# zfountas/deep-active-inference-mc

Measured on AMD Instinct MI355X. Metric: EFE rollouts/sec (64x64 dSprites, 10 MC-samples, depth 5), higher is better.
Workload: dtype f32; 1 GPU; calculate_G_repeated: 128 rows (32 roots x 4 actions) x depth 5 x 10 MC samples per GPU (BASELINE configs[1]) + action posterior; rows_per_gpu=128, samples=10, depth=5, parallelism=episodes sharded x1, weights replicated

## Files before the change

deep-active-inference-mc_amd/csrc/decoder.hip:

```cpp
#include <utility>
#include "mfma_pipe.h"

namespace efe {

template <class F, int... I> __device__ __forceinline__ void static_for_(F&& f, std::integer_sequence<int, I...>) { (f(std::integral_constant<int, I>{}), ...); }
template <int N, class F> __device__ __forceinline__ void static_for(F&& f) { static_for_(f, std::make_integer_sequence<int, N>{}); }

__host__ __device__ constexpr int w3_nch(int G) { return G == 4 ? 5 : 4; }
__host__ __device__ constexpr int w3_prod(int G, int c) {
    return G < 4 ? 5 * ((G >> 1) + 2 * (c >> 1)) + (G & 1) + 2 * (c & 1)
         : G == 4 ? (c < 2 ? 5 * (1 + 2 * c) + 4 : c < 4 ? 20 + 1 + 2 * (c - 2) : 24)
                  : (c < 2 ? 5 * (2 * c) + 4 : 20 + 2 * (c - 2));
}
__host__ __device__ constexpr bool w3_direct(int pp) { return f22_o1(pp / 5) < 0 && f22_o1(pp % 5) < 0; }
__host__ __device__ constexpr int w3_view(int pp) { return 3 * f22_view(pp / 5) + f22_view(pp % 5); }
__host__ __device__ constexpr int w3_mat(int pp) { return 4 * f22_wt(pp / 5) + f22_wt(pp % 5); }
__host__ __device__ constexpr bool w3_hits(int pp, int o) {
    const int r = o >> 2, c = o & 3, pr = pp / 5, pc = pp % 5;
    return (r == f22_o0(pr) || r == f22_o1(pr)) && (c == f22_o0(pc) || c == f22_o1(pc));
}
__host__ __device__ constexpr bool w3_seen(int G, int c, int o) {
    for (int g = 0; g < G; ++g)
        for (int k = 0; k < w3_nch(g); ++k) if (w3_hits(w3_prod(g, k), o)) return true;
    if (!w3_direct(w3_prod(G, c)))
        for (int k = 0; k < w3_nch(G); ++k)
            if ((w3_direct(w3_prod(G, k)) || k < c) && w3_hits(w3_prod(G, k), o)) return true;
    return false;
}
__host__ __device__ constexpr bool w3_uses_view(int G, int vi) {
    for (int k = 0; k < w3_nch(G); ++k) if (w3_view(w3_prod(G, k)) == vi) return true;
    return false;
}
__host__ __device__ constexpr bool f22_in(int a, int r) { return a == 0 ? r <= 1 : (a == 1 ? r == 1 : r >= 1); }
__host__ __device__ constexpr bool w3_reads(int G, int r, int c) {
    for (int vi = 0; vi < 9; ++vi) if (w3_uses_view(G, vi) && f22_in(vi / 3, r) && f22_in(vi % 3, c)) return true;
    return false;
}

constexpr int DA_PS = 17;
constexpr int DA_BIAS = 273 * DA_PS;

__host__ __device__ constexpr int wino_i0(int a) { return a == 0 ? 0 : (a == 2 ? 2 : 1); }
__host__ __device__ constexpr int wino_i1(int a) { return a == 0 ? 2 : (a == 1 ? 2 : (a == 2 ? 1 : 3)); }
__host__ __device__ constexpr float wino_s1(int a) { return a == 1 ? 1.0f : -1.0f; }
__host__ __device__ constexpr float wino_at(int r, int a) { return r == 0 ? (a < 3 ? 1.0f : 0.0f) : (a == 0 ? 0.0f : (a == 1 ? 1.0f : -1.0f)); }

template <int NR, int R0, class Pix>
__device__ __forceinline__ void wino_l1(f32x16 (&out)[NR][2], const float4* __restrict__ U, const float4* sm, const int h,
                                        const int mt_, Pix pix) {
    constexpr int PD = 4;
    const unsigned ln = (threadIdx.x & 63u) * 16u;
    const __amdgpu_buffer_rsrc_t ur = wrsrc(U);
    int mt = mt_; asm volatile("" : "+s"(mt));
    constexpr int a_lo = NR == 2 ? 0 : R0, a_hi = NR == 2 ? 4 : R0 + 3;
    auto ufrag = [&](int a, int b, int kc) { return wfrag(ur, ln, (size_t)(((4 * a + b) * 2 + mt) * 8 + kc) * 64); };
    auto bases = [&](int a, int b, int (&pb)[4]) {
        const int i0 = wino_i0(a), i1 = wino_i1(a), j0 = wino_i0(b), j1 = wino_i1(b);
        pb[0] = pix(i0, j0); pb[1] = pix(i0, j1); pb[2] = pix(i1, j0); pb[3] = pix(i1, j1);
    };
    float4 aq[PD], raw[4];
    int pb[4];
#pragma unroll
    for (int p = 0; p < PD; ++p) aq[p] = ufrag(a_lo, 0, p);
    bases(a_lo, 0, pb);
#pragma unroll
    for (int q = 0; q < 4; ++q) raw[q] = sm[pb[q] + h];
    f32x16 xacc;
    const f32x16 zero = {};
    auto otrans = [&](int a, int b, const f32x16& m, auto mask) {
        constexpr int MASK = decltype(mask)::value;
#pragma unroll
        for (int r = 0; r < NR; ++r) {
            if (!((MASK >> r) & 1)) continue;
            const float car = wino_at(R0 + r, a);
#pragma unroll
            for (int c = 0; c < 2; ++c) {
                const float cbc = wino_at(c, b);
                if (cbc == 0.0f) continue;
                const float cf = car * cbc;
#pragma unroll
                for (int e = 0; e < 16; ++e) out[r][c][e] = __builtin_fmaf(cf, m[e], out[r][c][e]);
            }
        }
    };
    auto xi_row = [&](int a, auto mask) {
        const float s1 = wino_s1(a);
        const int an = a + 1 < a_hi ? a + 1 : a;
#pragma unroll
        for (int b = 0; b < 4; ++b) {
            const float t1 = wino_s1(b);
#pragma unroll
            for (int kc = 0; kc < 8; ++kc) {
                const float4 av = aq[kc % PD];
                aq[kc % PD] = (b * 8 + kc + PD < 32) ? ufrag(a, (b * 8 + kc + PD) >> 3, (kc + PD) & 7) : ufrag(an, 0, (kc + PD) & 7);
                float4 v;
                {
                    const float4 c0 = make_float4(__builtin_fmaf(s1, raw[2].x, raw[0].x), __builtin_fmaf(s1, raw[2].y, raw[0].y),
                                                  __builtin_fmaf(s1, raw[2].z, raw[0].z), __builtin_fmaf(s1, raw[2].w, raw[0].w));
                    const float4 c1 = make_float4(__builtin_fmaf(s1, raw[3].x, raw[1].x), __builtin_fmaf(s1, raw[3].y, raw[1].y),
                                                  __builtin_fmaf(s1, raw[3].z, raw[1].z), __builtin_fmaf(s1, raw[3].w, raw[1].w));
                    v = make_float4(__builtin_fmaf(t1, c1.x, c0.x), __builtin_fmaf(t1, c1.y, c0.y), __builtin_fmaf(t1, c1.z, c0.z), __builtin_fmaf(t1, c1.w, c0.w));
                }
                if (kc < 7) {
#pragma unroll
                    for (int q = 0; q < 4; ++q) raw[q] = sm[pb[q] + 2 * (kc + 1) + h];
                } else {
                    if (b < 3) bases(a, b + 1, pb);
                    else bases(an, 0, pb);
#pragma unroll
                    for (int q = 0; q < 4; ++q) raw[q] = sm[pb[q] + h];
                }
                __builtin_amdgcn_sched_barrier(0);
                f32x16& x = xacc;
                x = __builtin_amdgcn_mfma_f32_32x32x2f32(av.x, v.x, kc == 0 ? zero : x, 0, 0, 0);
                x = __builtin_amdgcn_mfma_f32_32x32x2f32(av.y, v.y, x, 0, 0, 0);
                x = __builtin_amdgcn_mfma_f32_32x32x2f32(av.z, v.z, x, 0, 0, 0);
                x = __builtin_amdgcn_mfma_f32_32x32x2f32(av.w, v.w, x, 0, 0, 0);
            }
            otrans(a, b, xacc, mask);
        }
    };
    if constexpr (NR == 2) {
        xi_row(0, std::integral_constant<int, 1>{});
#pragma unroll 1
        for (int a = 1; a < 3; ++a) xi_row(a, std::integral_constant<int, 3>{});
        xi_row(3, std::integral_constant<int, 2>{});
    } else {
#pragma unroll 1
        for (int a = a_lo; a < a_hi; ++a) xi_row(a, std::integral_constant<int, 1>{});
    }
}
struct F22Nb { int xb, c2[3], r2; };
__device__ __forceinline__ f32x4 f22_wfrag(const __amdgpu_buffer_rsrc_t wr, const unsigned ln, int ct, int m, int kc) {
    return __builtin_bit_cast(f32x4, wfrag(wr, ln + (unsigned)kc * 1024u, (size_t)(m * 4 + ct) * 256));
}
constexpr int F22_PD = 2;
__device__ __forceinline__ void f22_l2_first(f32x4 (&aq)[F22_PD][5], const __amdgpu_buffer_rsrc_t wr, const int dn, const unsigned ln) {
    static_for<F22_PD>([&](auto p) {
        static_for<w3_nch(p >> 2)>([&](auto c) { aq[p][c] = f22_wfrag(wr, ln, dn, w3_mat(w3_prod(p >> 2, c)), p & 3); });
    });
}
__device__ __forceinline__ void f22_l2(f32x4 (&acc)[16], f32x4 (&aq)[F22_PD][5], const __amdgpu_buffer_rsrc_t wr, const int dn,
                                       const unsigned ln, const f32x4 bias4, const f32x4* smv, const F22Nb& nb) {
    constexpr int NST = 24;
    auto px = [&](int i, int jj, int kc) -> f32x4 {
        return smv[(jj == 2 ? nb.c2[i] : (i == 2 ? nb.r2 + jj * DA_PS : nb.xb + (16 * i + jj) * DA_PS)) + 4 * kc];
    };
    auto view = [&](const f32x4 (&x)[9], int vi) -> f32x4 {
        const int va = vi / 3, vb = vi % 3;
        auto cv = [&](int i) -> f32x4 { return vb == 0 ? x[3 * i] - x[3 * i + 1] : (vb == 1 ? x[3 * i + 1] : x[3 * i + 2] - x[3 * i + 1]); };
        return va == 0 ? cv(0) - cv(1) : (va == 1 ? cv(1) : cv(2) - cv(1));
    };
    const f32x4 zero4 = {};
    f32x4 tq[5], xr[9];
    static_for<9>([&](auto i) { if constexpr (w3_reads(0, i / 3, i % 3)) xr[i] = px(i / 3, i % 3, 0); });
    static_for<NST>([&](auto stc) {
        constexpr int ST = decltype(stc)::value, G = ST >> 2, KC = ST & 3, GN = (ST + 1) >> 2, KN = (ST + 1) & 3;
        constexpr int SP = (ST + F22_PD) % NST, GP = SP >> 2, KP = SP & 3;
        f32x4 vw[9], ac[5];
        static_for<9>([&](auto vi) { if constexpr (w3_uses_view(G, vi)) vw[vi] = view(xr, vi); });
#pragma unroll
        for (int c = 0; c < 5; ++c) ac[c] = aq[ST % F22_PD][c];
        static_for<w3_nch(GP)>([&](auto c) { aq[ST % F22_PD][c] = f22_wfrag(wr, ln, ST + F22_PD < NST ? 0 : dn, w3_mat(w3_prod(GP, c)), KP); });
        if constexpr (ST + 1 < NST)
            static_for<9>([&](auto i) { if constexpr (w3_reads(GN, i / 3, i % 3)) xr[i] = px(i / 3, i % 3, KN); });
        __builtin_amdgcn_sched_barrier(0);
#pragma unroll
        for (int e = 0; e < 4; ++e)
            static_for<w3_nch(G)>([&](auto c) {
                constexpr int PP = w3_prod(G, c);
                const float b = vw[w3_view(PP)][e], av = ac[c][e];
                if constexpr (w3_direct(PP)) {
                    constexpr int O = 4 * f22_o0(PP / 5) + f22_o0(PP % 5);
                    constexpr bool FIRST = KC == 0 && !w3_seen(G, c, O);
                    acc[O] = __builtin_amdgcn_mfma_f32_16x16x4f32(av, b, (FIRST && e == 0) ? bias4 : acc[O], 0, 0, 0);
                } else {
                    tq[c] = __builtin_amdgcn_mfma_f32_16x16x4f32(av, b, (KC == 0 && e == 0) ? zero4 : tq[c], 0, 0, 0);
                }
            });
        if constexpr (KC == 3)
            static_for<w3_nch(G)>([&](auto c) {
                constexpr int PP = w3_prod(G, c);
                if constexpr (!w3_direct(PP))
                    static_for<16>([&](auto o) {
                        if constexpr (w3_hits(PP, o)) {
                            if constexpr (w3_seen(G, c, o)) acc[o] = acc[o] + tq[c];
                            else acc[o] = bias4 + tq[c];
                        }
                    });
            });
    });
}
__device__ __forceinline__ void f22_l2_store(f32x4 (&acc)[16], const __amdgpu_buffer_rsrc_t yr, const unsigned yoff, const int ct, const bool on) {
#pragma unroll
    for (int orow = 0; orow < 4; ++orow)
#pragma unroll
        for (int c = 0; c < 2; ++c) {
            u32x4 lo, hi;
#pragma unroll
            for (int e = 0; e < 4; ++e) {
                const unsigned x0 = __builtin_bit_cast(unsigned, relu_nan(acc[4 * orow + c][e]));
                const unsigned x1 = __builtin_bit_cast(unsigned, relu_nan(acc[4 * orow + c + 2][e]));
                const auto sw = __builtin_amdgcn_permlane32_swap(x0, x1, false, false);
                lo[e] = sw[0]; hi[e] = sw[1];
            }
            const unsigned so = (unsigned)(((2 * (orow & 1) + c) * 4096 + 2 * ct * 512 + (orow >> 1) * 32) * 16);
            if (on) {
                __builtin_amdgcn_raw_buffer_store_b128(lo, yr, yoff, so, 0);
                __builtin_amdgcn_raw_buffer_store_b128(hi, yr, yoff, so + 512u * 16u, 0);
            }
        }
}

__global__ void __launch_bounds__(256, 2) k_dec_a(const DecAArgs a) {
    constexpr int NTHR = 256;
    constexpr int NPH = 2048 / NTHR;
    constexpr int NPE = 8;
    extern __shared__ __attribute__((aligned(16))) float4 sm[];
    const int tid = threadIdx.x;
    const int lane = tid & 63;
    const int w = __builtin_amdgcn_readfirstlane(tid >> 6);

    const float4* W1 = reinterpret_cast<const float4*>(a.w1);
    const float4* W2 = reinterpret_cast<const float4*>(a.w2);

    if ((int)blockIdx.x >= a.rows) return;
    int* const slot = reinterpret_cast<int*>(sm + DA_BIAS + 32);
    if (tid == 0) slot[0] = 2 * (int)gridDim.x + atomicAdd(a.queue, 1);
    int nimg = (int)blockIdx.x + (int)gridDim.x;
    f32x4 pf[2 * NPH];
    f32x4* smv = reinterpret_cast<f32x4*>(sm);
    {
        const f32x4* X = reinterpret_cast<const f32x4*>(a.x4) + (size_t)blockIdx.x * 4096;
#pragma unroll
        for (int it = 0; it < 2 * NPH; ++it) pf[it] = X[w * 1024 + it * 64 + lane];
    }
    for (int i = tid; i < 17 * DA_PS; i += NTHR) sm[256 * DA_PS + i] = make_float4(0.f, 0.f, 0.f, 0.f);
    if (tid < 16) sm[DA_BIAS + tid] = reinterpret_cast<const float4*>(a.b1)[tid];
    else if (tid < 32) sm[DA_BIAS + tid] = reinterpret_cast<const float4*>(a.b2)[tid - 16];

    for (int img = blockIdx.x; img < a.rows;) {
        int tl_ = tid; asm volatile("" : "+v"(tl_));
        const int j = tl_ & 31, h = (tl_ >> 5) & 1;
        const bool live = row_live(a.live, img);
        if (live) {
            const int sbase = (64 * w + ((tl_ >> 4) & 3)) * DA_PS + (tl_ & 15);
#pragma unroll
            for (int it = 0; it < 2 * NPH; ++it) smv[sbase + it * 4 * DA_PS] = pf[it];
        }
        __syncthreads();
        const int nnimg = slot[0];
        int ticket = 0;
        if (tid == 0) ticket = 2 * (int)gridDim.x + atomicAdd(a.queue, 1);
        const int l1mt = w >> 1, l1n = 32 * (w & 1) + j;
        const int l1y = 2 * (l1n >> 3) - 1, l1x = 2 * (l1n & 7) - 1;
        if (live) {
            f32x16 l1o[2][2];
#pragma unroll
            for (int g4 = 0; g4 < 4; ++g4) {
                const float4 bb = sm[DA_BIAS + l1mt * 8 + 2 * g4 + h];
#pragma unroll
                for (int rc = 0; rc < 4; ++rc) { l1o[rc >> 1][rc & 1][4 * g4] = bb.x; l1o[rc >> 1][rc & 1][4 * g4 + 1] = bb.y; l1o[rc >> 1][rc & 1][4 * g4 + 2] = bb.z; l1o[rc >> 1][rc & 1][4 * g4 + 3] = bb.w; }
            }
            wino_l1<2, 0>(l1o, W1, sm, h, l1mt, [&](int i, int jj) {
                const int y = l1y + i, x = l1x + jj;
                return ((unsigned)y < 16u && (unsigned)x < 16u ? y * 16 + x : 256) * DA_PS;
            });
            __syncthreads();
            if (tid == 0) slot[0] = ticket;
#pragma unroll
            for (int rc = 0; rc < 4; ++rc) {
                const int pix = (l1y + 1 + (rc >> 1)) * 16 + l1x + 1 + (rc & 1);
#pragma unroll
                for (int g4 = 0; g4 < 4; ++g4) {
                    const f32x16& o = l1o[rc >> 1][rc & 1];
                    float4 v;
                    v.x = relu_nan(o[4 * g4 + 0]); v.y = relu_nan(o[4 * g4 + 1]);
                    v.z = relu_nan(o[4 * g4 + 2]); v.w = relu_nan(o[4 * g4 + 3]);
                    sm[pix * DA_PS + l1mt * 8 + 2 * g4 + h] = v;
                }
            }
        } else {
            __syncthreads();
            if (tid == 0) slot[0] = ticket;
        }
        __syncthreads();
        {
            int t2_ = tid; asm volatile("" : "+v"(t2_));
            const int n = t2_ & 15, g = (t2_ >> 4) & 3;
            const int bu = 2 * w + (n >> 3), bv = n & 7;
            const int zq = 256 * DA_PS + g;
            F22Nb nb;
            nb.xb = (32 * bu + 2 * bv) * DA_PS + g;
            nb.c2[0] = bv == 7 ? zq : nb.xb + 2 * DA_PS;
            nb.c2[1] = bv == 7 ? zq : nb.xb + 18 * DA_PS;
            nb.c2[2] = bv == 7 ? zq : nb.xb + 34 * DA_PS;
            nb.r2 = nb.xb + 32 * DA_PS;
            const unsigned ln = (unsigned)(t2_ & 63) * 16u;
            const unsigned yoff = (unsigned)(((32 * bu + 2 * bv + (g >> 1)) * 2 + (g & 1)) * 16);
            const __amdgpu_buffer_rsrc_t yr = wrsrc(a.y2 + (size_t)__builtin_amdgcn_readfirstlane(img) * (32 * 32 * 64));
            auto load_next = [&](const int lo, const int hi) {
                const int pimg = __builtin_amdgcn_readfirstlane(nimg < a.rows ? nimg : img);
                const __amdgpu_buffer_rsrc_t xr = wrsrc(a.x4 + (size_t)pimg * 16384);
#pragma unroll
                for (int it = 0; it < 2 * NPH; ++it)
                    if (it >= lo && it < hi) pf[it] = __builtin_bit_cast(f32x4, wfrag(xr, (unsigned)(w * 16384 + (t2_ & 63) * 16 + (it & 3) * 1024), (size_t)(it >> 2) * 256));
            };
            if (live) {
                f32x4 aq[F22_PD][5], acc2[16];
                f22_l2_first(aq, wrsrc(W2), 0, ln);
                load_next(0, NPE);
#pragma unroll 1
                for (int ct = 0; ct < 4; ++ct) {
                    const f32x4 bias4 = smv[DA_BIAS + 16 + 4 * ct + g];
                    f22_l2(acc2, aq, wrsrc(W2 + ct * 256), ct < 3 ? 1 : 0, ln, bias4, smv, nb);
                    if (ct < 3) f22_l2_store(acc2, yr, yoff, ct, true);
                }
                load_next(NPE, 2 * NPH);
                f22_l2_store(acc2, yr, yoff, 3, true);
            } else {
                load_next(0, 2 * NPH);
            }
        }
        __syncthreads();
        img = nimg; nimg = nnimg;
    }
}

constexpr int DAS_IN = 6 * 16;
constexpr int DAS_L1 = 4 * 16;
constexpr int DAS_BIAS = (DAS_IN + 1 + DAS_L1 + 2) * DA_PS;
constexpr size_t DAS_LDS_BYTES = (DAS_BIAS + 32) * sizeof(float4);
__global__ void __launch_bounds__(256, 2) k_dec_a_s(const DecAArgs a) {
    extern __shared__ __attribute__((aligned(16))) float4 sm[];
    float4* sin = sm;
    float4* sl1 = sm + (DAS_IN + 1) * DA_PS;
    const int tid = threadIdx.x, lane = tid & 63;
    const int w = __builtin_amdgcn_readfirstlane(tid >> 6);
    const int j = lane & 31, h = lane >> 5;
    const int img = blockIdx.x >> 3, p = blockIdx.x & 7;
    if (!row_live(a.live, img)) return;
    const float4* W1 = reinterpret_cast<const float4*>(a.w1);
    const float4* W2 = reinterpret_cast<const float4*>(a.w2);
    {
        const float4* X = reinterpret_cast<const float4*>(a.x4) + (size_t)img * 4096;
        const int c4 = tid & 15, px0 = tid >> 4;
        float4 v[6];
#pragma unroll
        for (int it = 0; it < 6; ++it) {
            const int pix = px0 + 16 * it, lr = pix >> 4, y = 2 * p - 1 + lr;
            v[it] = (y >= 0 && y < 16) ? X[(y * 16 + (pix & 15)) * 16 + c4] : make_float4(0.f, 0.f, 0.f, 0.f);
        }
#pragma unroll
        for (int it = 0; it < 6; ++it) sin[(px0 + 16 * it) * DA_PS + c4] = v[it];
    }
    if (tid < 16) sin[DAS_IN * DA_PS + tid] = make_float4(0.f, 0.f, 0.f, 0.f);
    if (tid < 2 * DA_PS) sl1[DAS_L1 * DA_PS + tid] = make_float4(0.f, 0.f, 0.f, 0.f);
    if (tid < 16) sm[DAS_BIAS + tid] = reinterpret_cast<const float4*>(a.b1)[tid];
    else if (tid < 32) sm[DAS_BIAS + tid] = reinterpret_cast<const float4*>(a.b2)[tid - 16];
    __syncthreads();
    const int mt = w >> 1;
    {
        const int r = w & 1, n = j & 15;
        const int ly = 2 * (n >> 3) - 1, lx = 2 * (n & 7) - 1;
        f32x16 o[1][2];
#pragma unroll
        for (int g4 = 0; g4 < 4; ++g4) {
            const float4 bb = sm[DAS_BIAS + mt * 8 + 2 * g4 + h];
#pragma unroll
            for (int c = 0; c < 2; ++c) { o[0][c][4 * g4] = bb.x; o[0][c][4 * g4 + 1] = bb.y; o[0][c][4 * g4 + 2] = bb.z; o[0][c][4 * g4 + 3] = bb.w; }
        }
        auto pix = [&](int i, int jj) {
            const int sy = ly + 1 + i, x = lx + jj, y = 2 * p - 1 + sy;
            return ((unsigned)y < 16u && (unsigned)x < 16u ? sy * 16 + x : DAS_IN) * DA_PS;
        };
        if (r) wino_l1<1, 1>(o, W1, sin, h, mt, pix);
        else wino_l1<1, 0>(o, W1, sin, h, mt, pix);
        if (j < 16)
#pragma unroll
        for (int c = 0; c < 2; ++c)
#pragma unroll
            for (int g4 = 0; g4 < 4; ++g4) {
                float4 v;
                v.x = relu_nan(o[0][c][4 * g4 + 0]); v.y = relu_nan(o[0][c][4 * g4 + 1]);
                v.z = relu_nan(o[0][c][4 * g4 + 2]); v.w = relu_nan(o[0][c][4 * g4 + 3]);
                sl1[((ly + 1 + r) * 16 + lx + 1 + c) * DA_PS + mt * 8 + 2 * g4 + h] = v;
            }
    }
    __syncthreads();
    {
        const int n = lane & 15, g = lane >> 4, bv = n & 7;
        const int zq = DAS_L1 * DA_PS + g;
        F22Nb nb;
        nb.xb = 2 * bv * DA_PS + g;
        nb.c2[0] = bv == 7 ? zq : nb.xb + 2 * DA_PS;
        nb.c2[1] = bv == 7 ? zq : nb.xb + 18 * DA_PS;
        nb.c2[2] = (bv == 7 || p == 7) ? zq : nb.xb + 34 * DA_PS;
        nb.r2 = p == 7 ? zq : nb.xb + 32 * DA_PS;
        const unsigned ln = (unsigned)lane * 16u;
        const unsigned yoff = (unsigned)(((32 * p + 2 * bv + (g >> 1)) * 2 + (g & 1)) * 16);
        const __amdgpu_buffer_rsrc_t yr = wrsrc(a.y2 + (size_t)img * (32 * 32 * 64));
        const __amdgpu_buffer_rsrc_t wr = wrsrc(W2 + w * 256);
        f32x4 aq[F22_PD][5], acc2[16];
        f22_l2_first(aq, wr, 0, ln);
        const f32x4 bias4 = reinterpret_cast<const f32x4*>(sm)[DAS_BIAS + 16 + 4 * w + g];
        f22_l2(acc2, aq, wr, 0, ln, bias4, reinterpret_cast<const f32x4*>(sl1), nb);
        f22_l2_store(acc2, yr, yoff, w, n < 8);
    }
}

constexpr size_t DA_LDS_BYTES = (DA_BIAS + 33) * sizeof(float4);
int init_dec_b_kernels();
int init_decoder_kernels() {
    if (hipFuncSetAttribute((const void*)k_dec_a, hipFuncAttributeMaxDynamicSharedMemorySize, DA_LDS_BYTES) != hipSuccess) return 1;
    if (hipFuncSetAttribute((const void*)k_dec_a_s, hipFuncAttributeMaxDynamicSharedMemorySize, DAS_LDS_BYTES) != hipSuccess) return 1;
    return init_dec_b_kernels();
}

void launch_dec_a(const DecAArgs& a, hipStream_t st) {
    if (a.parts == 8) {
        hipLaunchKernelGGL(k_dec_a_s, dim3(a.rows * 8), dim3(256), DAS_LDS_BYTES, st, a);
        return;
    }
    const size_t lds = DA_LDS_BYTES;
    const int grid = a.rows < 512 ? a.rows : 512;
    hipLaunchKernelGGL(k_dec_a, dim3(grid), dim3(256), lds, st, a);
}


template <int PARTS>
__global__ void __launch_bounds__(256, 2) k_dec_b4(const DecBArgs a) {
    constexpr int SR = 4, NW = 4, NTHR = 256;
    constexpr int DB_RP = 33;
    constexpr int DB_PS = 17;
    constexpr int DB_IN_F4 = (SR + 1) * DB_RP * DB_PS;
    constexpr int DB_YROWS = 4 * SR + 2;
    constexpr int NPF = (SR + 1) * 512 / NTHR;
    constexpr int NS = 32 / SR;
    constexpr int NST = 24;
    extern __shared__ __attribute__((aligned(16))) float4 sm[];
    float* sH = reinterpret_cast<float*>(sm + DB_IN_F4);
    __shared__ float4 sb3[8];
    const int tid = threadIdx.x;
    const int lane = tid & 63;
    const int w = __builtin_amdgcn_readfirstlane(tid >> 6);
    const int g = lane >> 4, v = lane & 15;
    const int u = w >> 1, hf = w & 1;
    constexpr int parts = PARTS;
    const int img = parts == 1 ? (int)blockIdx.x : (int)(blockIdx.x >> 2);
    const int qtr = parts == 1 ? 0 : (int)(blockIdx.x & 3);
    if (!row_live(a.live, img)) return;
    const int s_lo = parts == 1 ? 0 : (qtr ? 2 * qtr - 1 : 0);
    const int s_hi = parts == 1 ? NS : 2 * qtr + 2;

    const int mg = a.m0 + img;
    const int gi = mg / a.rows_per_group;
    const int r = mg - gi * a.rows_per_group;
    int gt, gp, gs;
    group_decode(a.gm, gi, gt, gp, gs);
    const int mode = (gp == 0 && a.reward0) ? 1 : 0;
    const int slot = (gp == 0 && a.store0) ? gt * a.gm.S + gs : -1;
    float* po = (slot >= 0) ? a.po + ((size_t)slot * a.rows_per_group + r) * 4096 : nullptr;

    __shared__ float sq[4 * NTHR];
    __shared__ float sQ[4];
    if (tid < 8) sb3[tid] = reinterpret_cast<const float4*>(a.b3)[tid];
    if (tid < (SR + 1) * 16) sm[((tid >> 4) * DB_RP + 32) * DB_PS + (tid & 15)] = make_float4(0.f, 0.f, 0.f, 0.f);
    f32x4 w4a;
    {
        const int kh = v >> 2, kw = v & 3;
#pragma unroll
        for (int rr = 0; rr < 4; ++rr) w4a[rr] = (kh < 3 && kw < 3) ? a.w4[(3 * kh + kw) * 32 + 16 * hf + 4 * g + rr] : 0.f;
    }

    const __amdgpu_buffer_rsrc_t xr = __builtin_amdgcn_make_buffer_rsrc(const_cast<float*>(a.y2) + (size_t)img * (32 * 32 * 64), 0, 32 * 32 * 64 * 4, 0x00020000);
    const __amdgpu_buffer_rsrc_t wr = wrsrc(a.w3 + (size_t)hf * 4 * 64 * 4);
    const unsigned ln = (unsigned)lane * 16u;
    auto wf = [&](int m, int kc) -> f32x4 { return __builtin_bit_cast(f32x4, wfrag(wr, ln, (size_t)(m * 8 + kc) * 64)); };
    const float D1 = 1.00001f, D0 = 0.00001f;
    float part = 0.f;
    f32x4 pf[NPF];
    f32x4* smv = reinterpret_cast<f32x4*>(sm);
    auto prefetch = [&](int sn, int tl) {
        const unsigned lo = (unsigned)(((tl >> 5) * 512 + (tl & 31)) * 16);
        const unsigned lh = lo | (sn == NS - 1 ? 0x80000000u : 0u);
#pragma unroll
        for (int it = 0; it < NPF; ++it) {
            const int rl = it >> 1;
            const unsigned pc = (unsigned)((((rl & 1) * 16 + (it & 1) * 8) * 512 + (rl >> 1) * 32) * 16);
            pf[it] = __builtin_bit_cast(f32x4, __builtin_amdgcn_raw_buffer_load_b128(xr, rl == SR ? lh : lo, pc + (unsigned)sn * 1024u, 0));
        }
    };
    prefetch(s_lo, tid);

    const int xb = (2 * u * DB_RP + 2 * v) * DB_PS + g;
    auto px = [&](int i, int jj, int kc) -> f32x4 { return smv[xb + (i * DB_RP + jj) * DB_PS + 4 * kc]; };
    auto view = [&](const f32x4 (&x)[9], int vi) -> f32x4 {
        const int va = vi / 3, vb = vi % 3;
        auto cv = [&](int i) -> f32x4 { return vb == 0 ? sub4(x[3 * i], x[3 * i + 1]) : (vb == 1 ? x[3 * i + 1] : sub4(x[3 * i + 2], x[3 * i + 1])); };
        return va == 0 ? sub4(cv(0), cv(1)) : (va == 1 ? cv(1) : sub4(cv(2), cv(1)));
    };

    constexpr int RWG = 2 * SR / NW;
    float gh[RWG][6], gpr[RWG];
    auto g_load = [&](int oh, int q, int r0y, int hb0) {
#pragma unroll
        for (int kh = 0; kh < 3; ++kh) {
            const int tr = oh + 1 - kh;
            const bool rv = tr >= 0 && tr <= 63;
            int hs = hb0 + (tr - r0y);
            hs = hs < 0 ? hs + DB_YROWS : hs;
            hs = hs >= DB_YROWS ? hs - DB_YROWS : hs;
            hs = rv ? hs : 0;
            const float* hq = sH + ((hs * 2) * 3 + kh) * 64 + lane;
            gh[q][2 * kh] = hq[0]; gh[q][2 * kh + 1] = hq[3 * 64];
        }
    };
    auto g_sig = [&](int oh, int q) {
        float val = a.b4;
#pragma unroll
        for (int kh = 0; kh < 3; ++kh) {
            const int tr = oh + 1 - kh;
            val = add1(val, (tr >= 0 && tr <= 63) ? add1(gh[q][2 * kh], gh[q][2 * kh + 1]) : 0.f);
        }
        gpr[q] = hw_sigmoid(val);
    };
    auto g_term = [&](int oh, int q) {
#pragma clang fp contract(off)
        const float pr = gpr[q];
        const float l1 = hw_log(D1 - pr), l0 = hw_log(D0 + pr);
        const float te = __builtin_fmaf(pr - 1.0f, l1, -(pr * l0));
        const float tw = reward_term(pr, oh, lane, 64, 64, a.reward_intent);
        const float t = mode == 0 ? te : tw;
        part += oh >= 0 ? t : 0.0f;
    };
    auto g_store = [&](int oh, int q) {
        if (po && oh >= 0) {
            int owl = lane; asm volatile("" : "+v"(owl));
            (po + oh * 64)[owl] = gpr[q];
        }
    };

    auto fold = [&](int k) { sq[k * NTHR + tid] = part; part = 0.f; };
    float* const sHw = sH + g * 64 + 4 * v;
    int hb = 0, hbp = 0;
    for (int s = s_lo; s < s_hi; ++s) {
        int tl = tid; asm volatile("" : "+v"(tl));
        const bool gq = parts == 1 ? true : s == 2 * qtr + 1;
        const int oh0 = 2 * SR * (s - 1) - 1 + w, oh1 = oh0 + NW;
        {
            f32x4* const sp = smv + ((tl & 31) >> 1) * (2 * DB_PS) + 2 * (tl >> 5) + (tl & 1);
#pragma unroll
            for (int it = 0; it < NPF; ++it) sp[((it >> 1) * DB_RP + (it & 1)) * DB_PS] = pf[it];
        }
        f32x4 aq[5];
#pragma unroll
        for (int c = 0; c < w3_nch(0); ++c) aq[c] = wf(w3_mat(w3_prod(0, c)), 0);
        __syncthreads();

        const f32x4 bias4 = __builtin_bit_cast(f32x4, sb3[4 * hf + g]);
        const f32x4 zero4 = {};
        f32x4 acc[16], tq[5];
        f32x4 xr[9];
        static_for<9>([&](auto i) { if constexpr (w3_reads(0, i / 3, i % 3)) xr[i] = px(i / 3, i % 3, 0); });
        static_for<NST>([&](auto stc) {
            constexpr int ST = decltype(stc)::value, G = ST >> 2, KC = ST & 3, GN = (ST + 1) >> 2, KN = (ST + 1) & 3;
            f32x4 vw[9], ac[5];
            static_for<9>([&](auto vi) { if constexpr (w3_uses_view(G, vi)) vw[vi] = view(xr, vi); });
#pragma unroll
            for (int c = 0; c < 5; ++c) ac[c] = aq[c];
            if constexpr (ST + 1 < NST) {
                static_for<w3_nch(GN)>([&](auto c) { aq[c] = wf(w3_mat(w3_prod(GN, c)), KN); });
                static_for<9>([&](auto i) { if constexpr (w3_reads(GN, i / 3, i % 3)) xr[i] = px(i / 3, i % 3, KN); });
            }
            __builtin_amdgcn_sched_barrier(0);
#pragma unroll
            for (int e = 0; e < 4; ++e)
                static_for<w3_nch(G)>([&](auto c) {
                    constexpr int PP = w3_prod(G, c);
                    const float b = vw[w3_view(PP)][e], av = ac[c][e];
                    if constexpr (w3_direct(PP)) {
                        constexpr int O = 4 * f22_o0(PP / 5) + f22_o0(PP % 5);
                        constexpr bool FIRST = KC == 0 && !w3_seen(G, c, O);
                        acc[O] = __builtin_amdgcn_mfma_f32_16x16x4f32(av, b, (FIRST && e == 0) ? bias4 : acc[O], 0, 0, 0);
                    } else {
                        tq[c] = __builtin_amdgcn_mfma_f32_16x16x4f32(av, b, (KC == 0 && e == 0) ? zero4 : tq[c], 0, 0, 0);
                    }
                });
            if constexpr (KC == 3)
                static_for<w3_nch(G)>([&](auto c) {
                    constexpr int PP = w3_prod(G, c);
                    if constexpr (!w3_direct(PP))
                        static_for<16>([&](auto o) {
                            if constexpr (w3_hits(PP, o)) {
                                if constexpr (w3_seen(G, c, o)) acc[o] = add4(acc[o], tq[c]);
                                else acc[o] = add4(bias4, tq[c]);
                            }
                        });
                });
            if (gq) {
                if constexpr (ST == 0) { g_load(oh0, 0, 2 * SR * (s - 1), hbp); g_load(oh1, 1, 2 * SR * (s - 1), hbp); }
                if constexpr (ST == 2) g_sig(oh0, 0);
                if constexpr (ST == 5) g_term(oh0, 0);
                if constexpr (ST == 8) g_sig(oh1, 1);
                if constexpr (ST == 11) g_term(oh1, 1);
            }
        });
        prefetch((s < NS - 1) ? s + 1 : NS - 1, tl);
#pragma unroll
        for (int orow = 0; orow < 4; ++orow) {
            f32x4 T[4];
#pragma unroll
            for (int oc = 0; oc < 4; ++oc)
#pragma unroll
                for (int e = 0; e < 4; ++e) acc[4 * orow + oc][e] = relu_nan(acc[4 * orow + oc][e]);
#pragma unroll
            for (int e = 0; e < 4; ++e)
#pragma unroll
                for (int oc = 0; oc < 4; ++oc)
                    T[oc] = __builtin_amdgcn_mfma_f32_16x16x4f32(w4a[e], acc[4 * orow + oc][e], e == 0 ? zero4 : T[oc], 0, 0, 0);
            f32x4 hv;
            hv[0] = add1(add1(T[1][0], T[0][1]), dpp_shr1_zero(T[3][2]));
            hv[1] = add1(add1(T[2][0], T[1][1]), T[0][2]);
            hv[2] = add1(add1(T[3][0], T[2][1]), T[1][2]);
            hv[3] = add1(add1(dpp_shl1_zero(T[0][0]), T[3][1]), T[2][2]);
            int hsw = hb + 4 * u + orow;
            hsw = hsw >= DB_YROWS ? hsw - DB_YROWS : hsw;
            if (g < 3) *reinterpret_cast<f32x4*>(sHw + (hsw * 2 + hf) * (3 * 64)) = hv;
        }
        __syncthreads();
        if (gq) { g_store(oh0, 0); g_store(oh1, 1); }
        if (parts == 1 && (s == 2 || s == 4 || s == 6)) fold(s / 2 - 1);
        if (s == s_hi - 1) {
#pragma unroll
            for (int q = 0; q <= RWG; ++q) {
                if (q == RWG && (w != 0 || s != NS - 1)) break;
                const int oh = 2 * SR * s - 1 + q * NW + w;
                g_load(oh, 0, 2 * SR * s, hb); g_sig(oh, 0); g_term(oh, 0); g_store(oh, 0);
            }
        }
        hbp = hb;
        hb += 2 * SR;
        hb = hb >= DB_YROWS ? hb - DB_YROWS : hb;
    }
    fold(parts == 1 ? 3 : 0);
    __syncthreads();
    if (w < (parts == 1 ? 4 : 1)) {
        const float* qk = sq + w * NTHR + lane;
        float val = add1(add1(qk[0], qk[64]), add1(qk[128], qk[192]));
#pragma unroll
        for (int o = 32; o > 0; o >>= 1) val += __shfl_xor(val, o);
        if (lane == 0) sQ[w] = val;
    }
    __syncthreads();
    if (tid == 0) {
        if (parts == 1) a.val[mg] = add1(add1(sQ[0], sQ[1]), add1(sQ[2], sQ[3]));
        else a.valq[(size_t)mg * 4 + qtr] = sQ[0];
    }
}

constexpr size_t DB_LDS4D = ((5 * 33) * 17) * sizeof(float4) + 18 * 2 * 3 * 64 * sizeof(float);
int init_dec_b_kernels() {
    if (hipFuncSetAttribute((const void*)k_dec_b4<1>, hipFuncAttributeMaxDynamicSharedMemorySize, DB_LDS4D) != hipSuccess) return 1;
    if (hipFuncSetAttribute((const void*)k_dec_b4<4>, hipFuncAttributeMaxDynamicSharedMemorySize, DB_LDS4D) != hipSuccess) return 1;
    return 0;
}

void launch_dec_b(const DecBArgs& a, hipStream_t st) {
    if (a.parts == 4) hipLaunchKernelGGL(k_dec_b4<4>, dim3(a.rows * 4), dim3(256), DB_LDS4D, st, a);
    else hipLaunchKernelGGL(k_dec_b4<1>, dim3(a.rows), dim3(256), DB_LDS4D, st, a);
}

__host__ __device__ inline int fc4_spg(int mtiles) { return ((mtiles + 7) / 8 + 7) / 8; }
template <int NT>
__global__ void __launch_bounds__(256, 2) k_fc4(const GemmArgs a) {
    constexpr int RT = 32 * NT;
    extern __shared__ __attribute__((aligned(16))) float4 sm[];
    const int tid = threadIdx.x;
    const int lane = tid & 63;
    const int w = __builtin_amdgcn_readfirstlane(tid >> 6);
    const int j = lane & 31, h = lane >> 5;
    const int fgrp = blockIdx.x & 7;
    const int nper = gridDim.x >> 3, k = blockIdx.x >> 3;
    const int SPG = fc4_spg(a.mtiles);
    const int nsteps = ((a.n_pix + RT - 1) / RT) * SPG;
    const int q0 = (int)(((long)nsteps * k) / nper), q1 = (int)(((long)nsteps * (k + 1)) / nper);
    f32x4* smv = reinterpret_cast<f32x4*>(sm);
    const float4* Wl = reinterpret_cast<const float4*>(a.Wp);
    auto xaddr = [&](int t, int (&bs)[NT], int (&sw)[NT], int& wt) {
        wt = t;
#pragma unroll
        for (int nt = 0; nt < NT; ++nt) { bs[nt] = (nt * 32 + j) * 64 + t * 16; sw[nt] = j & 15; }
    };
    int cur_rt = -1;
    uint32_t krow[2] = {0, 0}, kstream[2] = {0, 0}, kstage[2] = {0, 0};
    bool rv[2] = {false, false};
#pragma unroll 1
    for (int q = q0; q < q1; ++q) {
        const int rt = q / SPG, fs = q - rt * SPG;
        const int row0 = rt * RT;
        if (rt != cur_rt) {
            if (cur_rt >= 0) __syncthreads();
            cur_rt = rt;
            const f32x4* X = reinterpret_cast<const f32x4*>(a.X);
#pragma unroll
            for (int it = 0; it < 8 * NT; ++it) {
                const int idx = it * 256 + tid;
                const int r = idx >> 6, c4 = idx & 63;
                const int gr = row0 + r;
                smv[r * 64 + (c4 ^ (r & 15))] = (gr < a.n_pix) ? X[(size_t)gr * 64 + c4] : (f32x4)(0.f);
            }
            __syncthreads();
#pragma unroll
            for (int nt = 0; nt < NT; ++nt) {
                const int m = row0 + nt * 32 + j;
                rv[nt] = m < a.n_pix;
                const int mg = a.m0 + (rv[nt] ? m : 0);
                const int g = mg / a.rows_per_group;
                krow[nt] = global_row(a.gm.ids, a.gm.ids_div, mg - g * a.rows_per_group, a.row_offset);
                const uint2 key = group_key(a.gm, g);
                kstream[nt] = key.x; kstage[nt] = key.y;
            }
        }
        const int mt0 = (fgrp * SPG + fs) * 8 + 2 * w;
        if (mt0 >= a.mtiles) continue;
        f32x16 acc[2][NT];
#pragma unroll
        for (int mt = 0; mt < 2; ++mt)
#pragma unroll
            for (int nt = 0; nt < NT; ++nt)
#pragma unroll
                for (int e = 0; e < 16; ++e) acc[mt][nt][e] = 0.f;
        float4 bq[2][4];
#pragma unroll
        for (int mt = 0; mt < 2; ++mt)
#pragma unroll
            for (int g4 = 0; g4 < 4; ++g4) bq[mt][g4] = *reinterpret_cast<const float4*>(a.bias + (mt0 + mt) * 32 + 8 * g4 + 4 * h);
        tap_loop<2, NT>(acc, 4, Wl, sm, h, xaddr, DenseWIdx{mt0});
#pragma unroll
        for (int nt = 0; nt < NT; ++nt) {
            if (!rv[nt]) continue;
            const uint4 rnd = noise_words(a.k0, a.k1, a.tag, (uint32_t)((mt0 * 32) >> 7), krow[nt], kstream[nt], kstage[nt]);
            float* yp = a.Y + (size_t)(row0 + nt * 32 + j) * a.ldy;
#pragma unroll
            for (int mt = 0; mt < 2; ++mt)
#pragma unroll
                for (int g4 = 0; g4 < 4; ++g4) {
                    const int co = (mt0 + mt) * 32 + 8 * g4 + 4 * h;
                    const float4 bb = bq[mt][g4];
                    const uint32_t word = ((co >> 5) & 3) == 0 ? rnd.x : ((co >> 5) & 3) == 1 ? rnd.y : ((co >> 5) & 3) == 2 ? rnd.z : rnd.w;
                    float v[4] = {acc[mt][nt][4 * g4 + 0] + bb.x, acc[mt][nt][4 * g4 + 1] + bb.y,
                                  acc[mt][nt][4 * g4 + 2] + bb.z, acc[mt][nt][4 * g4 + 3] + bb.w};
#pragma unroll
                    for (int e = 0; e < 4; ++e) v[e] = relu_nan(v[e]) * keep2(((word >> ((co + e) & 31)) & 1u));
                    *reinterpret_cast<float4*>(yp + co) = make_float4(v[0], v[1], v[2], v[3]);
                }
        }
    }
}

void launch_fc4(const GemmArgs& a, hipStream_t st) {
    if (a.n_pix <= 32) {
        const int nsteps = fc4_spg(a.mtiles);
        hipLaunchKernelGGL(k_fc4<1>, dim3(8 * (nsteps < 64 ? nsteps : 64)), dim3(256), 32 * 64 * sizeof(float4), st, a);
        return;
    }
    const int nsteps = ((a.n_pix + 63) / 64) * fc4_spg(a.mtiles);
    const int nper = nsteps < 64 ? nsteps : 64;
    hipLaunchKernelGGL(k_fc4<2>, dim3(8 * nper), dim3(256), 64 * 64 * sizeof(float4), st, a);
}

}
```

deep-active-inference-mc_amd/csrc/mfma_pipe.h:

```cpp
#pragma once
#include "kernels.h"

#ifndef EFE_PD_WIDE
#define EFE_PD_WIDE 1
#endif
#ifndef EFE_PD_NARROW
#define EFE_PD_NARROW 2
#endif

namespace efe {

typedef float f32x16 __attribute__((ext_vector_type(16)));
typedef float f32x2 __attribute__((ext_vector_type(2)));
typedef float f32x4 __attribute__((ext_vector_type(4)));

#define MFMA4(ACC, AV, BV)                                                      \
    ACC = __builtin_amdgcn_mfma_f32_32x32x2f32((AV).x, (BV).x, ACC, 0, 0, 0);   \
    ACC = __builtin_amdgcn_mfma_f32_32x32x2f32((AV).y, (BV).y, ACC, 0, 0, 0);   \
    ACC = __builtin_amdgcn_mfma_f32_32x32x2f32((AV).z, (BV).z, ACC, 0, 0, 0);   \
    ACC = __builtin_amdgcn_mfma_f32_32x32x2f32((AV).w, (BV).w, ACC, 0, 0, 0);

#define MFMA4I(ACC, INIT, AV, BV)                                               \
    ACC = __builtin_amdgcn_mfma_f32_32x32x2f32((AV).x, (BV).x, INIT, 0, 0, 0);  \
    ACC = __builtin_amdgcn_mfma_f32_32x32x2f32((AV).y, (BV).y, ACC, 0, 0, 0);   \
    ACC = __builtin_amdgcn_mfma_f32_32x32x2f32((AV).z, (BV).z, ACC, 0, 0, 0);   \
    ACC = __builtin_amdgcn_mfma_f32_32x32x2f32((AV).w, (BV).w, ACC, 0, 0, 0);

typedef unsigned u32x4 __attribute__((ext_vector_type(4)));
__device__ __forceinline__ __amdgpu_buffer_rsrc_t wrsrc(const void* base) {
    return __builtin_amdgcn_make_buffer_rsrc(const_cast<void*>(base), 0, 0x7fffffff, 0x00020000);
}
__device__ __forceinline__ float4 wfrag(__amdgpu_buffer_rsrc_t r, unsigned lane_bytes, size_t f4_index) {
    const u32x4 v = __builtin_amdgcn_raw_buffer_load_b128(r, lane_bytes, (unsigned)f4_index * 16u, 0);
    return __builtin_bit_cast(float4, v);
}

#define EFE_OPAQUE(r) asm("" : "+v"(r))
__device__ __forceinline__ float add1(float a, float b) { float r = a + b; EFE_OPAQUE(r); return r; }
__device__ __forceinline__ float sub1(float a, float b) { EFE_OPAQUE(b); float r = a - b; EFE_OPAQUE(r); return r; }
__device__ __forceinline__ f32x4 add4(f32x4 a, f32x4 b) {
    f32x4 r;
#pragma unroll
    for (int e = 0; e < 4; ++e) r[e] = add1(a[e], b[e]);
    return r;
}
__device__ __forceinline__ f32x4 sub4(f32x4 a, f32x4 b) {
    f32x4 r;
#pragma unroll
    for (int e = 0; e < 4; ++e) r[e] = sub1(a[e], b[e]);
    return r;
}


__device__ __forceinline__ float hw_sigmoid(float v) { return __builtin_amdgcn_rcpf(1.0f + __builtin_amdgcn_exp2f(v * -1.4426950408889634f)); }
__device__ __forceinline__ float hw_log(float x) { return __builtin_amdgcn_logf(x) * 0.6931471805599453f; }

__device__ __forceinline__ float dpp_shr1_zero(float x) { return __builtin_bit_cast(float, __builtin_amdgcn_update_dpp(0, __builtin_bit_cast(int, x), 0x111, 0xf, 0xf, true)); }
__device__ __forceinline__ float dpp_shl1_zero(float x) { return __builtin_bit_cast(float, __builtin_amdgcn_update_dpp(0, __builtin_bit_cast(int, x), 0x101, 0xf, 0xf, true)); }
__device__ __forceinline__ float dpp_shr1_keep(float old, float x) { return __builtin_bit_cast(float, __builtin_amdgcn_update_dpp(__builtin_bit_cast(int, old), __builtin_bit_cast(int, x), 0x111, 0xf, 0xf, false)); }
__device__ __forceinline__ float dpp_shl1_keep(float old, float x) { return __builtin_bit_cast(float, __builtin_amdgcn_update_dpp(__builtin_bit_cast(int, old), __builtin_bit_cast(int, x), 0x101, 0xf, 0xf, false)); }
__device__ __forceinline__ float wave_shr1(float x) { return __builtin_bit_cast(float, __builtin_amdgcn_update_dpp(0, __builtin_bit_cast(int, x), 0x138, 0xf, 0xf, true)); }
__device__ __forceinline__ float wave_shl1(float x) { return __builtin_bit_cast(float, __builtin_amdgcn_update_dpp(0, __builtin_bit_cast(int, x), 0x130, 0xf, 0xf, true)); }
__device__ __forceinline__ float dpp_ror1(float x) { return __builtin_bit_cast(float, __builtin_amdgcn_update_dpp(0, __builtin_bit_cast(int, x), 0x121, 0xf, 0xf, false)); }
__device__ __forceinline__ float dpp_ror15(float x) { return __builtin_bit_cast(float, __builtin_amdgcn_update_dpp(0, __builtin_bit_cast(int, x), 0x12f, 0xf, 0xf, false)); }



struct DenseWIdx {
    int mt0;
    template <int MT> __device__ __forceinline__ size_t at(int wt, int mt, int kc) const { return (size_t)((mt0 + mt) * 32 + wt * 8 + kc) * 64; }
};

template <int MT, int NT, int KC = 8, int PD = 1>
struct TapPipe {
    static_assert(KC % PD == 0, "the A-fragment ring must wrap consistently across taps");
    float4 aq[PD][MT];
    float4 bv[NT];
    int bs[NT], sw[NT], wt;

    template <class AddrFn, class WIdx>
    __device__ __forceinline__ void begin(const float4* __restrict__ Wl, const float4* sm, const int h, AddrFn addr, WIdx widx) {
        const unsigned ln = (threadIdx.x & 63u) * 16u;
        const __amdgpu_buffer_rsrc_t wr = wrsrc(Wl);
        addr(0, bs, sw, wt);
#pragma unroll
        for (int p = 0; p < PD; ++p)
#pragma unroll
            for (int mt = 0; mt < MT; ++mt) aq[p][mt] = wfrag(wr, ln, widx.template at<MT>(wt, mt, p));
#pragma unroll
        for (int nt = 0; nt < NT; ++nt) bv[nt] = sm[bs[nt] + (h ^ sw[nt])];
    }

    template <class AddrFn, class WIdx>
    __device__ __forceinline__ void run(f32x16 (&acc)[MT][NT], const int ntaps, const float4* __restrict__ Wl,
                                        const float4* sm, const int h, AddrFn addr, WIdx widx) {
        const unsigned ln = (threadIdx.x & 63u) * 16u;
        const __amdgpu_buffer_rsrc_t wr = wrsrc(Wl);
        for (int t = 0; t < ntaps; ++t) {
            int nbs[NT], nsw[NT], nwt;
            addr((t + 1 < ntaps) ? t + 1 : t, nbs, nsw, nwt);
#pragma unroll
            for (int kc = 0; kc < KC; ++kc) {
                float4 av[MT], bn[NT];
#pragma unroll
                for (int mt = 0; mt < MT; ++mt) av[mt] = aq[kc % PD][mt];
#pragma unroll
                for (int mt = 0; mt < MT; ++mt)
                    aq[kc % PD][mt] = (kc + PD < KC) ? wfrag(wr, ln, widx.template at<MT>(wt, mt, kc + PD))
                                                     : wfrag(wr, ln, widx.template at<MT>(nwt, mt, kc + PD - KC));
                if (kc < KC - 1) {
#pragma unroll
                    for (int nt = 0; nt < NT; ++nt) bn[nt] = sm[bs[nt] + ((2 * (kc + 1) + h) ^ sw[nt])];
                } else {
#pragma unroll
                    for (int nt = 0; nt < NT; ++nt) bn[nt] = sm[nbs[nt] + (h ^ nsw[nt])];
                }
                __builtin_amdgcn_sched_barrier(0);
#pragma unroll
                for (int mt = 0; mt < MT; ++mt)
#pragma unroll
                    for (int nt = 0; nt < NT; ++nt) { MFMA4(acc[mt][nt], av[mt], bv[nt]) }
#pragma unroll
                for (int nt = 0; nt < NT; ++nt) bv[nt] = bn[nt];
            }
#pragma unroll
            for (int nt = 0; nt < NT; ++nt) { bs[nt] = nbs[nt]; sw[nt] = nsw[nt]; }
            wt = nwt;
        }
    }
};

template <int MT, int NT, class AddrFn, class WIdx>
__device__ __forceinline__ void tap_loop(f32x16 (&acc)[MT][NT], const int ntaps, const float4* __restrict__ Wl,
                                         const float4* sm, const int h, AddrFn addr, WIdx widx) {
    TapPipe<MT, NT, 8, (MT * NT >= 4 ? EFE_PD_WIDE : EFE_PD_NARROW)> p;
    p.begin(Wl, sm, h, addr, widx);
    p.run(acc, ntaps, Wl, sm, h, addr, widx);
}


template <int MT, int NT, int KC, class AddrFn, class WIdx>
__device__ __forceinline__ void tap_loop_kc(f32x16 (&acc)[MT][NT], const int ntaps, const float4* __restrict__ Wl,
                                            const float4* sm, const int h, AddrFn addr, WIdx widx) {
    TapPipe<MT, NT, KC, EFE_PD_NARROW> p;
    p.begin(Wl, sm, h, addr, widx);
    p.run(acc, ntaps, Wl, sm, h, addr, widx);
}

template <int MT, int NT, int KC, int PD, class AddrFn, class WIdx>
__device__ __forceinline__ void tap_loop_kc_pd(f32x16 (&acc)[MT][NT], const int ntaps, const float4* __restrict__ Wl,
                                               const float4* sm, const int h, AddrFn addr, WIdx widx) {
    TapPipe<MT, NT, KC, PD> p;
    p.begin(Wl, sm, h, addr, widx);
    p.run(acc, ntaps, Wl, sm, h, addr, widx);
}

struct PackedWIdx {
    int mtiles, kcn, mt0;
    template <int MT> __device__ __forceinline__ size_t at(int wt, int mt, int kc) const {
        return (size_t)((wt * mtiles + mt0 + mt) * kcn + kc) * 64;
    }
};

}
```

Before: 11810 rollouts/s.

## Add wave priority hints, defer tmp adds, and software-pipeline decoder final-layer MFMAs

```diff
diff --git a/deep-active-inference-mc_amd/csrc/decoder.hip b/deep-active-inference-mc_amd/csrc/decoder.hip
--- a/deep-active-inference-mc_amd/csrc/decoder.hip
+++ b/deep-active-inference-mc_amd/csrc/decoder.hip
@@ -110,12 +110,14 @@
 #pragma unroll
                     for (int q = 0; q < 4; ++q) raw[q] = sm[pb[q] + h];
                 }
+                prio_matrix();
                 __builtin_amdgcn_sched_barrier(0);
                 f32x16& x = xacc;
                 x = __builtin_amdgcn_mfma_f32_32x32x2f32(av.x, v.x, kc == 0 ? zero : x, 0, 0, 0);
                 x = __builtin_amdgcn_mfma_f32_32x32x2f32(av.y, v.y, x, 0, 0, 0);
                 x = __builtin_amdgcn_mfma_f32_32x32x2f32(av.z, v.z, x, 0, 0, 0);
                 x = __builtin_amdgcn_mfma_f32_32x32x2f32(av.w, v.w, x, 0, 0, 0);
+                prio_nonmatrix();
             }
             otrans(a, b, xacc, mask);
         }
@@ -164,6 +166,7 @@
         static_for<w3_nch(GP)>([&](auto c) { aq[ST % F22_PD][c] = f22_wfrag(wr, ln, ST + F22_PD < NST ? 0 : dn, w3_mat(w3_prod(GP, c)), KP); });
         if constexpr (ST + 1 < NST)
             static_for<9>([&](auto i) { if constexpr (w3_reads(GN, i / 3, i % 3)) xr[i] = px(i / 3, i % 3, KN); });
+        prio_matrix();
         __builtin_amdgcn_sched_barrier(0);
 #pragma unroll
         for (int e = 0; e < 4; ++e)
@@ -178,6 +181,7 @@
                     tq[c] = __builtin_amdgcn_mfma_f32_16x16x4f32(av, b, (KC == 0 && e == 0) ? zero4 : tq[c], 0, 0, 0);
                 }
             });
+        prio_nonmatrix();
         if constexpr (KC == 3)
             static_for<w3_nch(G)>([&](auto c) {
                 constexpr int PP = w3_prod(G, c);
@@ -503,26 +507,26 @@
 
     constexpr int RWG = 2 * SR / NW;
     float gh[RWG][6], gpr[RWG];
-    auto g_load = [&](int oh, int q, int r0y, int hb0) {
+    constexpr unsigned HROW = 2 * 3 * 64 * sizeof(float), HRING = DB_YROWS * HROW;
+    auto ring_fwd = [&](unsigned o, unsigned rows) { o += rows * HROW; const unsigned t = o - HRING; return t < o ? t : o; };
+    const float* const sHl = sH + lane;
+    unsigned gm[RWG][3];
+    auto g_load = [&](unsigned go, int q) {
 #pragma unroll
         for (int kh = 0; kh < 3; ++kh) {
-            const int tr = oh + 1 - kh;
-            const bool rv = tr >= 0 && tr <= 63;
-            int hs = hb0 + (tr - r0y);
-            hs = hs < 0 ? hs + DB_YROWS : hs;
-            hs = hs >= DB_YROWS ? hs - DB_YROWS : hs;
-            hs = rv ? hs : 0;
-            const float* hq = sH + ((hs * 2) * 3 + kh) * 64 + lane;
+            const float* hq = reinterpret_cast<const float*>(reinterpret_cast<const char*>(sHl) + (kh == 2 ? go : ring_fwd(go, 2 - kh))) + kh * 64;
             gh[q][2 * kh] = hq[0]; gh[q][2 * kh + 1] = hq[3 * 64];
         }
     };
-    auto g_sig = [&](int oh, int q) {
+    auto g_mask = [&](int oh, int q) {
+#pragma unroll
+        for (int kh = 0; kh < 3; ++kh) gm[q][kh] = (unsigned)(oh + 1 - kh) <= 63u ? ~0u : 0u;
+    };
+    auto g_sig = [&](int q) {
         float val = a.b4;
 #pragma unroll
-        for (int kh = 0; kh < 3; ++kh) {
-            const int tr = oh + 1 - kh;
-            val = add1(val, (tr >= 0 && tr <= 63) ? add1(gh[q][2 * kh], gh[q][2 * kh + 1]) : 0.f);
-        }
+        for (int kh = 0; kh < 3; ++kh)
+            val = add1(val, __builtin_bit_cast(float, __builtin_bit_cast(unsigned, add1(gh[q][2 * kh], gh[q][2 * kh + 1])) & gm[q][kh]));
         gpr[q] = hw_sigmoid(val);
     };
     auto g_term = [&](int oh, int q) {
@@ -542,14 +546,17 @@
     };
 
     auto fold = [&](int k) { sq[k * NTHR + tid] = part; part = 0.f; };
-    float* const sHw = sH + g * 64 + 4 * v;
-    int hb = 0, hbp = 0;
+    char* const sHw = reinterpret_cast<char*>(sH + hf * (3 * 64) + g * 64 + 4 * v);
+    unsigned hbo = 0;
+    const int tl = tid;
+    f32x4* const sp = smv + ((tl & 31) >> 1) * (2 * DB_PS) + 2 * (tl >> 5) + (tl & 1);
     for (int s = s_lo; s < s_hi; ++s) {
-        int tl = tid; asm volatile("" : "+v"(tl));
         const bool gq = parts == 1 ? true : s == 2 * qtr + 1;
         const int oh0 = 2 * SR * (s - 1) - 1 + w, oh1 = oh0 + NW;
+        const unsigned go0 = ring_fwd(hbo, DB_YROWS - 2 * SR - 2 + w), go1 = ring_fwd(go0, NW);
+        const unsigned hwo = ring_fwd(hbo, 4 * u);
+        g_mask(oh0, 0); g_mask(oh1, 1);
         {
-            f32x4* const sp = smv + ((tl & 31) >> 1) * (2 * DB_PS) + 2 * (tl >> 5) + (tl & 1);
 #pragma unroll
             for (int it = 0; it < NPF; ++it) sp[((it >> 1) * DB_RP + (it & 1)) * DB_PS] = pf[it];
         }
@@ -563,6 +570,19 @@
         f32x4 acc[16], tq[5];
         f32x4 xr[9];
         static_for<9>([&](auto i) { if constexpr (w3_reads(0, i / 3, i % 3)) xr[i] = px(i / 3, i % 3, 0); });
+        auto add_tmp = [&](auto gg) {
+            constexpr int GG = decltype(gg)::value;
+            static_for<w3_nch(GG)>([&](auto c) {
+                constexpr int PP = w3_prod(GG, c);
+                if constexpr (!w3_direct(PP))
+                    static_for<16>([&](auto o) {
+                        if constexpr (w3_hits(PP, o)) {
+                            if constexpr (w3_seen(GG, c, o)) acc[o] = add4(acc[o], tq[c]);
+                            else acc[o] = add4(bias4, tq[c]);
+                        }
+                    });
+            });
+        };
         static_for<NST>([&](auto stc) {
             constexpr int ST = decltype(stc)::value, G = ST >> 2, KC = ST & 3, GN = (ST + 1) >> 2, KN = (ST + 1) & 3;
             f32x4 vw[9], ac[5];
@@ -573,6 +593,11 @@
                 static_for<w3_nch(GN)>([&](auto c) { aq[c] = wf(w3_mat(w3_prod(GN, c)), KN); });
                 static_for<9>([&](auto i) { if constexpr (w3_reads(GN, i / 3, i % 3)) xr[i] = px(i / 3, i % 3, KN); });
             }
+            if constexpr (KC == 0 && ST > 0) {
+                __builtin_amdgcn_sched_barrier(0);
+                add_tmp(std::integral_constant<int, (ST > 0 ? G - 1 : 0)>{});
+            }
+            prio_matrix();
             __builtin_amdgcn_sched_barrier(0);
 #pragma unroll
             for (int e = 0; e < 4; ++e)
@@ -587,47 +612,45 @@
                         tq[c] = __builtin_amdgcn_mfma_f32_16x16x4f32(av, b, (KC == 0 && e == 0) ? zero4 : tq[c], 0, 0, 0);
                     }
                 });
-            if constexpr (KC == 3)
-                static_for<w3_nch(G)>([&](auto c) {
-                    constexpr int PP = w3_prod(G, c);
-                    if constexpr (!w3_direct(PP))
-                        static_for<16>([&](auto o) {
-                            if constexpr (w3_hits(PP, o)) {
-                                if constexpr (w3_seen(G, c, o)) acc[o] = add4(acc[o], tq[c]);
-                                else acc[o] = add4(bias4, tq[c]);
-                            }
-                        });
-                });
+            prio_nonmatrix();
             if (gq) {
-                if constexpr (ST == 0) { g_load(oh0, 0, 2 * SR * (s - 1), hbp); g_load(oh1, 1, 2 * SR * (s - 1), hbp); }
-                if constexpr (ST == 2) g_sig(oh0, 0);
+                if constexpr (ST == 0) { g_load(go0, 0); g_load(go1, 1); }
+                if constexpr (ST == 2) g_sig(0);
                 if constexpr (ST == 5) g_term(oh0, 0);
-                if constexpr (ST == 8) g_sig(oh1, 1);
+                if constexpr (ST == 8) g_sig(1);
                 if constexpr (ST == 11) g_term(oh1, 1);
             }
         });
         prefetch((s < NS - 1) ? s + 1 : NS - 1, tl);
-#pragma unroll
-        for (int orow = 0; orow < 4; ++orow) {
-            f32x4 T[4];
+        auto relu_row = [&](int orow) {
 #pragma unroll
             for (int oc = 0; oc < 4; ++oc)
 #pragma unroll
                 for (int e = 0; e < 4; ++e) acc[4 * orow + oc][e] = relu_nan(acc[4 * orow + oc][e]);
-#pragma unroll
-            for (int e = 0; e < 4; ++e)
-#pragma unroll
-                for (int oc = 0; oc < 4; ++oc)
-                    T[oc] = __builtin_amdgcn_mfma_f32_16x16x4f32(w4a[e], acc[4 * orow + oc][e], e == 0 ? zero4 : T[oc], 0, 0, 0);
+        };
+        auto presum_row = [&](const f32x4 (&T)[4], int orow) {
             f32x4 hv;
             hv[0] = add1(add1(T[1][0], T[0][1]), dpp_shr1_zero(T[3][2]));
             hv[1] = add1(add1(T[2][0], T[1][1]), T[0][2]);
             hv[2] = add1(add1(T[3][0], T[2][1]), T[1][2]);
             hv[3] = add1(add1(dpp_shl1_zero(T[0][0]), T[3][1]), T[2][2]);
-            int hsw = hb + 4 * u + orow;
-            hsw = hsw >= DB_YROWS ? hsw - DB_YROWS : hsw;
-            if (g < 3) *reinterpret_cast<f32x4*>(sHw + (hsw * 2 + hf) * (3 * 64)) = hv;
-        }
+            if (g < 3) *reinterpret_cast<f32x4*>(sHw + ring_fwd(hwo, orow)) = hv;
+        };
+        f32x4 T[2][4];
+        relu_row(0);
+#pragma unroll
+        for (int orow = 0; orow < 4; ++orow) {
+            __builtin_amdgcn_sched_barrier(0);
+#pragma unroll
+            for (int e = 0; e < 4; ++e)
+#pragma unroll
+                for (int oc = 0; oc < 4; ++oc)
+                    T[orow & 1][oc] = __builtin_amdgcn_mfma_f32_16x16x4f32(w4a[e], acc[4 * orow + oc][e], e == 0 ? zero4 : T[orow & 1][oc], 0, 0, 0);
+            if (orow < 3) relu_row(orow + 1);
+            if (orow > 0) presum_row(T[(orow - 1) & 1], orow - 1);
+        }
+        __builtin_amdgcn_sched_barrier(0);
+        presum_row(T[1], 3);
         __syncthreads();
         if (gq) { g_store(oh0, 0); g_store(oh1, 1); }
         if (parts == 1 && (s == 2 || s == 4 || s == 6)) fold(s / 2 - 1);
@@ -636,12 +659,11 @@
             for (int q = 0; q <= RWG; ++q) {
                 if (q == RWG && (w != 0 || s != NS - 1)) break;
                 const int oh = 2 * SR * s - 1 + q * NW + w;
-                g_load(oh, 0, 2 * SR * s, hb); g_sig(oh, 0); g_term(oh, 0); g_store(oh, 0);
-            }
-        }
-        hbp = hb;
-        hb += 2 * SR;
-        hb = hb >= DB_YROWS ? hb - DB_YROWS : hb;
+                g_mask(oh, 0);
+                g_load(ring_fwd(ring_fwd(hbo, DB_YROWS - 2), q * NW + w), 0); g_sig(0); g_term(oh, 0); g_store(oh, 0);
+            }
+        }
+        hbo = ring_fwd(hbo, 2 * SR);
     }
     fold(parts == 1 ? 3 : 0);
     __syncthreads();
diff --git a/deep-active-inference-mc_amd/csrc/mfma_pipe.h b/deep-active-inference-mc_amd/csrc/mfma_pipe.h
--- a/deep-active-inference-mc_amd/csrc/mfma_pipe.h
+++ b/deep-active-inference-mc_amd/csrc/mfma_pipe.h
@@ -50,6 +50,9 @@
     for (int e = 0; e < 4; ++e) r[e] = sub1(a[e], b[e]);
     return r;
 }
+
+__device__ __forceinline__ void prio_nonmatrix() { __builtin_amdgcn_s_setprio(1); }
+__device__ __forceinline__ void prio_matrix() { __builtin_amdgcn_s_setprio(0); }
 
 
 __device__ __forceinline__ float hw_sigmoid(float v) { return __builtin_amdgcn_rcpf(1.0f + __builtin_amdgcn_exp2f(v * -1.4426950408889634f)); }
```

New measurement: 12030 rollouts/s, median of 6. +1.9%, better.
